# Peilun-Tommy-Li/pHNN-MPC

Measured on AMD Instinct MI355X. Metric: pHNN-MPC rollouts+grads/sec, cartpole H=50 batch=65536, higher is better.
Workload: dtype f32

## Files before the change

phnn_mpc_amd/csrc/phnn_kernels.hip.h:

```cpp
#pragma once
#include <hip/hip_runtime.h>

#include "../../include/phnn_mpc.h"

#define DEV __device__ __forceinline__
#ifdef PHNN_CACHED_TAPE
#define PHNN_NT_STORE(v, p) (*(p) = (v))
#define PHNN_NT_LOAD(p) (*(p))
#else
#define PHNN_NT_STORE(v, p) __builtin_nontemporal_store((v), (p))
#define PHNN_NT_LOAD(p) __builtin_nontemporal_load((p))
#endif

using f32x4 = __attribute__((ext_vector_type(4))) float;
using f32x2 = __attribute__((ext_vector_type(2))) float;

constexpr int kTileB = 16;
#ifndef PHNN_KMAXWAVES
#define PHNN_KMAXWAVES 8
#endif
constexpr int kMaxWaves = PHNN_KMAXWAVES;
constexpr int kScrFloats = 16 * 20;

struct Lane {
// ... 366 lines not shown
  f16x8 h[T / 2], l[T / 2];
};

template <int T>
DEV void split_act_h(const Act<T>& a, Split2<T>& o) {
#pragma unroll
  for (int s = 0; s < T / 2; ++s) {
    u32x4 H, Lo;
#pragma unroll
    for (int p = 0; p < 4; ++p) {
      f32x2 x = {a.v[2 * s + (p >> 1)][2 * (p & 1)], a.v[2 * s + (p >> 1)][2 * (p & 1) + 1]};
      f16x2 hb = __builtin_convertvector(x, f16x2);
      f32x2 r = residual_h(hb, x);
      H[p] = __builtin_bit_cast(unsigned, hb);
      Lo[p] = __builtin_bit_cast(unsigned, __builtin_convertvector(r, f16x2));
    }
    o.h[s] = __builtin_bit_cast(f16x8, H);
    o.l[s] = __builtin_bit_cast(f16x8, Lo);
  }
}

template <int HID>
struct HfImg {
  static constexpr int RS = HID + 16;
  static constexpr int PART = HID * RS * 2;
  static constexpr int FLOATS = 2 * PART / 4;
};

DEV f16x8 in_frag_h(f32x4 x) {
  f32x2 v01 = {x[0], x[1]}, v23 = {x[2], x[3]};
  f16x2 h01 = __builtin_convertvector(v01, f16x2), h23 = __builtin_convertvector(v23, f16x2);
  f32x2 r01 = residual_h(h01, v01), r23 = residual_h(h23, v23);
  u32x4 B = {__builtin_bit_cast(unsigned, h01), __builtin_bit_cast(unsigned, h23),
             __builtin_bit_cast(unsigned, __builtin_convertvector(r01, f16x2)),
             __builtin_bit_cast(unsigned, __builtin_convertvector(r23, f16x2))};
  return __builtin_bit_cast(f16x8, B);
}
constexpr int kInFragH(int T) { return T * 64 * 4; }
template <int T>
DEV void in_layer_h(Act<T>& o, const float* Wh, Lane ln, f16x8 xf) {
  keep_lds_reads_local();
#pragma unroll
  for (int nt = 0; nt < T; ++nt) o.v[nt] = mfma_h(*reinterpret_cast<const f16x8*>(Wh + (nt * 64 + ln.lane) * 4), xf, o.v[nt]);
}
constexpr int kInHFwd = 1, kInHRecomp = 2, kInHHvp = 4, kInHNet1 = 8, kInHNet1Adj = 16;
#ifndef PHNN_INH_MASK
#define PHNN_INH_MASK (kInHFwd | kInHRecomp | kInHHvp | kInHNet1 | kInHNet1Adj)
#endif
template <int T, int MM, int SITE>
DEV void in_layer_mm(Act<T>& o, const float* Lnet, int oF, int oFh, Lane ln, f32x4 x, int tile0 = 0) {
  if constexpr (MM == MM_F16X2 && (PHNN_INH_MASK & SITE) != 0) in_layer_h<T>(o, Lnet + oFh + tile0 * 256, ln, in_frag_h(x));
  else in_layer<T>(o, Lnet + oF + tile0 * 64, ln, sel4(x, ln.q));
}

DEV void mfma3x2(f32x4& o0, f32x4& o1, const f16x8 (&a)[2][2], f16x8 xh, f16x8 xl) {
  o0 = mfma_h(a[0][1], xh, o0);
  o1 = mfma_h(a[1][1], xh, o1);
  o0 = mfma_h(a[0][0], xl, o0);
  o1 = mfma_h(a[1][0], xl, o1);
  o0 = mfma_h(a[0][0], xh, o0);
  o1 = mfma_h(a[1][0], xh, o1);
}

template <int T>
DEV void sq_fwd_h(Act<T>& o, const float* Wimg, Lane ln, const Split2<T>& in) {
  using I = HfImg<16 * T>;
  keep_lds_reads_local();
  matrix_phase_begin();
  const char* base = reinterpret_cast<const char*>(Wimg) + ln.i * (I::RS * 2) + ln.q * 16;
#ifndef PHNN_NO_PREFETCH_FRAGS
  {
    constexpr int PD = 1, NB = PD + 1;
    f16x8 a[NB][2][2];
    auto loadg = [&](int g, f16x8 (&dst)[2][2]) {
      const int n0 = 2 * (g / (T / 2)), s = g % (T / 2);
#pragma unroll
      for (int gg = 0; gg < 2; ++gg)
#pragma unroll
        for (int p = 0; p < 2; ++p)
          dst[gg][p] = *reinterpret_cast<const f16x8*>(base + p * I::PART + (n0 + gg) * 16 * (I::RS * 2) + s * 64);
    };
    constexpr int NG = (T / 2) * (T / 2);
#pragma unroll
    for (int g = 0; g < PD && g < NG; ++g) loadg(g, a[g % NB]);
#pragma unroll
    for (int g = 0; g < NG; ++g) {
      if (g + PD < NG) loadg(g + PD, a[(g + PD) % NB]);
      __builtin_amdgcn_sched_barrier(0);
      const int n0 = 2 * (g / (T / 2)), s = g % (T / 2);
      mfma3x2(o.v[n0], o.v[n0 + 1], a[g % NB], in.h[s], in.l[s]);
      __builtin_amdgcn_sched_barrier(0);
    }
    matrix_phase_end();
    return;
  }
#endif
#pragma unroll
  for (int n0 = 0; n0 < T; n0 += 2) {
#pragma unroll
    for (int s = 0; s < T / 2; ++s) {
      f16x8 a[2][2];
#pragma unroll
      for (int g = 0; g < 2; ++g)
#pragma unroll
        for (int p = 0; p < 2; ++p)
          a[g][p] = *reinterpret_cast<const f16x8*>(base + p * I::PART + (n0 + g) * 16 * (I::RS * 2) + s * 64);
      mfma3x2(o.v[n0], o.v[n0 + 1], a, in.h[s], in.l[s]);
    }
  }
  matrix_phase_end();
}

template <int T>
DEV void sq_bwd_h(Act<T>& o, const float* Wimg, Lane ln, const Split2<T>& in) {
  using I = HfImg<16 * T>;
  keep_lds_reads_local();
  matrix_phase_begin();
  typedef fp16x4_t __attribute__((address_space(3))) * lds_h4;
  typedef char __attribute__((address_space(3))) * lds_cp;
  const int a4 = (ln.lane & 15) >> 2, pp = ln.lane & 3;
  lds_cp base = (lds_cp) const_cast<char*>(reinterpret_cast<const char*>(Wimg)) + (4 * ln.q + a4) * (I::RS * 2) + 16 * pp;
#ifndef PHNN_NO_PREFETCH_FRAGS
  {
    f16x8 a[2][2][2];
    auto loadg = [&](int g, f16x8 (&dst)[2][2]) {
      const int n0 = 2 * (g / (T / 2)), s = g % (T / 2);
#pragma unroll
      for (int gg = 0; gg < 2; ++gg) {
        const int nt = n0 + gg;
#pragma unroll
        for (int p = 0; p < 2; ++p) {
          lds_cp off = base + p * I::PART + 32 * s * (I::RS * 2) + (64 * (nt >> 1) + 8 * (nt & 1));
          f16x4 lo = __builtin_bit_cast(f16x4, __builtin_amdgcn_ds_read_tr16_b64_v4f16((lds_h4)off));
          f16x4 hi = __builtin_bit_cast(f16x4, __builtin_amdgcn_ds_read_tr16_b64_v4f16((lds_h4)(off + 16 * (I::RS * 2))));
          dst[gg][p] = __builtin_shufflevector(lo, hi, 0, 1, 2, 3, 4, 5, 6, 7);
        }
      }
    };
    constexpr int NG = (T / 2) * (T / 2);
    constexpr int PD = 1, NB = PD + 1;
#pragma unroll
    for (int g = 0; g < PD && g < NG; ++g) loadg(g, a[g % NB]);
#pragma unroll
    for (int g = 0; g < NG; ++g) {
      if (g + PD < NG) loadg(g + PD, a[(g + PD) % NB]);
      __builtin_amdgcn_sched_barrier(0);
      const int n0 = 2 * (g / (T / 2)), s = g % (T / 2);
      mfma3x2(o.v[n0], o.v[n0 + 1], a[g % NB], in.h[s], in.l[s]);
      __builtin_amdgcn_sched_barrier(0);
    }
    matrix_phase_end();
    return;
  }
#endif
#pragma unroll
  for (int n0 = 0; n0 < T; n0 += 2) {
#pragma unroll
    for (int s = 0; s < T / 2; ++s) {
      f16x8 a[2][2];
#pragma unroll
      for (int g = 0; g < 2; ++g) {
        const int nt = n0 + g;
#pragma unroll
        for (int p = 0; p < 2; ++p) {
          lds_cp off = base + p * I::PART + 32 * s * (I::RS * 2) + (64 * (nt >> 1) + 8 * (nt & 1));
          f16x4 lo = __builtin_bit_cast(f16x4, __builtin_amdgcn_ds_read_tr16_b64_v4f16((lds_h4)off));
          f16x4 hi = __builtin_bit_cast(f16x4, __builtin_amdgcn_ds_read_tr16_b64_v4f16((lds_h4)(off + 16 * (I::RS * 2))));
          a[g][p] = __builtin_shufflevector(lo, hi, 0, 1, 2, 3, 4, 5, 6, 7);
        }
      }
      mfma3x2(o.v[n0], o.v[n0 + 1], a, in.h[s], in.l[s]);
    }
  }
  matrix_phase_end();
}

template <int TG>
DEV f32x4 to4_group(const float* Wt_group, Lane ln, const f32x4* in_tiles) {
  const float* base = Wt_group + 4 * ln.q;
  f32x4 o0 = splat4(0.f), o1 = splat4(0.f);
#pragma unroll
  for (int t = 0; t < TG; ++t) {
    f32x4 a = *reinterpret_cast<const f32x4*>(base + 16 * t);
#pragma unroll
    for (int r = 0; r < 4; ++r) {
      if ((r & 1) == 0) o0 = __builtin_amdgcn_mfma_f32_4x4x1f32(a[r], in_tiles[t][r], o0, 0, 0, 0);
      else o1 = __builtin_amdgcn_mfma_f32_4x4x1f32(a[r], in_tiles[t][r], o1, 0, 0, 0);
    }
  }
  return o0 + o1;
}

DEV f32x4 to4_kslots(f32x4 o) {
#ifdef PHNN_BPERMUTE_REDUCE
#pragma unroll
  for (int c = 0; c < 4; ++c) {
    float v = o[c];
    v += __shfl_xor(v, 16);
    v += __shfl_xor(v, 32);
    o[c] = v;
  }
  return o;
#else
  f32x4 b;
  asm volatile("v_mov_b32 %4, %0\n\tv_mov_b32 %5, %1\n\tv_mov_b32 %6, %2\n\tv_mov_b32 %7, %3\n\t"
               "v_permlane16_swap_b32 %0, %4\n\tv_permlane16_swap_b32 %1, %5\n\t"
               "v_permlane16_swap_b32 %2, %6\n\tv_permlane16_swap_b32 %3, %7\n\ts_nop 0"
               : "+v"(o[0]), "+v"(o[1]), "+v"(o[2]), "+v"(o[3]), "=&v"(b[0]), "=&v"(b[1]), "=&v"(b[2]), "=&v"(b[3]));
  o = o + b;
  asm volatile("v_mov_b32 %4, %0\n\tv_mov_b32 %5, %1\n\tv_mov_b32 %6, %2\n\tv_mov_b32 %7, %3\n\t"
               "v_permlane32_swap_b32 %0, %4\n\tv_permlane32_swap_b32 %1, %5\n\t"
               "v_permlane32_swap_b32 %2, %6\n\tv_permlane32_swap_b32 %3, %7\n\ts_nop 0"
               : "+v"(o[0]), "+v"(o[1]), "+v"(o[2]), "+v"(o[3]), "=&v"(b[0]), "=&v"(b[1]), "=&v"(b[2]), "=&v"(b[3]));
  return o + b;
#endif
}

template <int TI>
DEV f32x4 to4_rep(const float* Wt, Lane ln, const Act<TI>& in) {
  constexpr int LR = 16 * TI + 8;
  keep_lds_reads_local();
  const float* row = Wt + (ln.i & 3) * LR;
  constexpr int TG = TI >= 2 ? 2 : 1, NG = TI / TG;
  f32x4 tot = to4_group<TG>(row, ln, &in.v[0]);
#pragma unroll
  for (int g = 1; g < NG; ++g) tot = tot + to4_group<TG>(row + 16 * TG * g, ln, &in.v[TG * g]);
  return to4_kslots(tot);
}

template <int T>
DEV void store_act(float* dst, Lane ln, const Act<T>& a) {
#pragma unroll
  for (int t = 0; t < T; ++t) PHNN_NT_STORE(a.v[t], reinterpret_cast<f32x4*>(dst) + t * 64 + ln.lane);
}
template <int T>
DEV void load_act(const float* src, Lane ln, Act<T>& a) {
#pragma unroll
  for (int t = 0; t < T; ++t) {
#ifdef PHNN_PLAIN_STASH_LOADS
    a.v[t] = reinterpret_cast<const f32x4*>(src)[t * 64 + ln.lane];
#else
    a.v[t] = PHNN_NT_LOAD(reinterpret_cast<const f32x4*>(src) + t * 64 + ln.lane);
#endif
  }
}

constexpr float kFix24 = 8388607.0f;
typedef unsigned u32x3 __attribute__((ext_vector_type(3), aligned(4)));
template <int T>
DEV void store_act24(float* dst, Lane ln, const Act<T>& a) {
#pragma unroll
  for (int t = 0; t < T; ++t) {
    unsigned q[4];
#pragma unroll
    for (int r = 0; r < 4; ++r) q[r] = (unsigned)(int)__builtin_rintf(a.v[t][r] * kFix24);
    u32x3 d = {__builtin_amdgcn_perm(q[1], q[0], 0x04020100u),
               __builtin_amdgcn_perm(q[2], q[1], 0x05040201u),
               __builtin_amdgcn_perm(q[3], q[2], 0x06050402u)};
    PHNN_NT_STORE(d, reinterpret_cast<u32x3*>(reinterpret_cast<char*>(dst) + (t * 64 + ln.lane) * 12));
  }
}
template <int T>
DEV void load_act24(const float* src, Lane ln, Act<T>& a) {
#pragma unroll
  for (int t = 0; t < T; ++t) {
    const u32x3 d = PHNN_NT_LOAD(reinterpret_cast<const u32x3*>(reinterpret_cast<const char*>(src) + (t * 64 + ln.lane) * 12));
    const int q0 = (int)(d[0] << 8) >> 8;
    const int q1 = (int)(__builtin_amdgcn_alignbit(d[1], d[0], 24) << 8) >> 8;
    const int q2 = (int)(__builtin_amdgcn_alignbit(d[2], d[1], 16) << 8) >> 8;
    const int q3 = (int)d[2] >> 8;
    a.v[t] = f32x4{(float)q0, (float)q1, (float)q2, (float)q3} * (1.0f / kFix24);
  }
}

DEV void gather16(float* scr, Lane ln, f32x4 mine, float (&out)[16]) {
  float* row = scr + ln.i * 20;
  *reinterpret_cast<f32x4*>(row + 4 * ln.q) = mine;
  __builtin_amdgcn_wave_barrier();
#pragma unroll
  for (int k = 0; k < 4; ++k) {
    f32x4 v = *reinterpret_cast<const f32x4*>(row + 4 * k);
    out[4 * k + 0] = v[0];
    out[4 * k + 1] = v[1];
    out[4 * k + 2] = v[2];
    out[4 * k + 3] = v[3];
  }
  __builtin_amdgcn_wave_barrier();
}

DEV float reduce_q(float v) {
#ifdef PHNN_BPERMUTE_REDUCE
  v += __shfl_xor(v, 16);
  v += __shfl_xor(v, 32);
  return v;
#else
  float b;
  asm volatile("v_mov_b32 %1, %0\n\ts_nop 1\n\tv_permlane16_swap_b32 %0, %1\n\ts_nop 0" : "+v"(v), "=&v"(b));
  v += b;
  asm volatile("v_mov_b32 %1, %0\n\ts_nop 1\n\tv_permlane32_swap_b32 %0, %1\n\ts_nop 0" : "+v"(v), "=&v"(b));
  return v + b;
#endif
}


template <int HID, int MM = MM_F32>
struct LayH2 {
  static constexpr int T = HID / 16, LD = HID + 4, LR = HID + 8;
  static constexpr int oW2 = 0;
  static constexpr int W2F = MM == MM_F32 ? HID * LD : (MM == MM_BF16X3 ? BfImg<HID>::FLOATS : HfImg<HID>::FLOATS);
  static constexpr int oW1h = oW2 + W2F;
  static constexpr int oW1f = oW1h + (MM == MM_F16X2 ? T * 64 * 4 : 0);
  static constexpr int oB1 = oW1f + T * 64;
  static constexpr int oB2 = oB1 + HID;
  static constexpr int oW3 = oB2 + HID;
  static constexpr int oW3B = oW3 + HID;
  static constexpr int oW3S = oW3B + HID;
  static constexpr int oW1T = oW3S + HID;
  static constexpr int oB3 = oW1T + 4 * LR;
  static constexpr int SIZE = oB3 + 4;
};

template <int HID, int MM = MM_F32>
struct LayH1 {
  static constexpr int T = HID / 16, LD = HID + 4, LR = HID + 8;
  static constexpr bool HF = MM == MM_F16X2;
  static constexpr int RS = HID + 16;
  static constexpr int FPART = 16 * RS * 2;
  static constexpr int BPART = HID * 16 * 2;
  static constexpr int oV2 = 0;
  static constexpr int oV2T = oV2 + 2 * FPART / 4;
  static constexpr int V2F = HF ? (2 * FPART + 2 * BPART) / 4 : 16 * LD;
  static constexpr int oV1h = oV2 + V2F;
  static constexpr int oV1f = oV1h + (HF ? T * 64 * 4 : 0);
  static constexpr int oC1 = oV1f + T * 64;
  static constexpr int oC2 = oC1 + HID;
  static constexpr int oSc = oC2 + 16;
  static constexpr int oV1T = oSc + 4;
  static constexpr int SIZE = oV1T + 4 * LR;
};

constexpr int kRecSmall = 40;
template <int T, int NBIG>
struct WRec {
  static constexpr int VEC = T * 256;
  static constexpr int oSmall = NBIG * VEC;
  static constexpr int SIZE = oSmall + 16 * kRecSmall;
};

#ifdef PHNN_CACHED_RECORDS
#define PHNN_REC_STORE(v, p) (*(p) = (v))
#define PHNN_REC_LOAD(p) (*(p))
#else
#define PHNN_REC_STORE(v, p) __builtin_nontemporal_store((v), (p))
#define PHNN_REC_LOAD(p) __builtin_nontemporal_load((p))
#endif
template <int T>
DEV void store_rec(float* dst, Lane ln, const Act<T>& a) {
#pragma unroll
  for (int t = 0; t < T; ++t) PHNN_REC_STORE(a.v[t], reinterpret_cast<f32x4*>(dst) + t * 64 + ln.lane);
}
template <int T>
DEV void store_rec_scaled(float* dst, Lane ln, const Act<T>& a, float s) {
#pragma unroll
  for (int t = 0; t < T; ++t) PHNN_REC_STORE(a.v[t] * s, reinterpret_cast<f32x4*>(dst) + t * 64 + ln.lane);
}

constexpr int ACT_TANH = 0, ACT_SILU = 2, ACT_RELU = 3, ACT_ELU = 4, ACT_GELU = 5;

DEV float gelu_pdf(float z) { return 0.3989422804014327f * __builtin_amdgcn_exp2f(z * z * -0.7213475204444817f); }
DEV float gelu_cdf(float z) { return __builtin_fmaf(0.5f, erff(z * 0.7071067811865476f), 0.5f); }

template <int ACT>
DEV void act_eval(float z, float& a, float& d1) {
  if (ACT == ACT_RELU) {
    a = fmaxf(z, 0.f);
    d1 = z > 0.f ? 1.0f : 0.0f;
  } else if (ACT == ACT_ELU) {
    a = z > 0.f ? z : expm1f(z);
    d1 = z > 0.f ? 1.0f : __builtin_amdgcn_exp2f(z * 1.4426950408889634f);
  } else if (ACT == ACT_GELU) {
    const float c = gelu_cdf(z);
    a = z * c;
    d1 = __builtin_fmaf(z, gelu_pdf(z), c);
  } else {
    const float s = __builtin_amdgcn_rcpf(1.0f + __builtin_amdgcn_exp2f(z * -1.4426950408889634f));
    a = z * s;
    d1 = __builtin_fmaf(a, 1.0f - s, s);
  }
}
template <int ACT>
DEV float act_d2(float z) {
  if (ACT == ACT_RELU) return 0.0f;
  if (ACT == ACT_ELU) return z > 0.f ? 0.0f : __builtin_amdgcn_exp2f(z * 1.4426950408889634f);
  if (ACT == ACT_GELU) return gelu_pdf(z) * __builtin_fmaf(-z, z, 2.0f);
  const float s = __builtin_amdgcn_rcpf(1.0f + __builtin_amdgcn_exp2f(z * -1.4426950408889634f));
  return s * (1.0f - s) * __builtin_fmaf(z, 1.0f - 2.0f * s, 2.0f);
}
template <int ACT, int T>
DEV void act_of(const Act<T>& z, Act<T>& a) {
#pragma unroll
  for (int t = 0; t < T; ++t)
#pragma unroll
    for (int r = 0; r < 4; ++r) {
      float av, d;
      act_eval<ACT>(z.v[t][r], av, d);
      a.v[t][r] = av;
    }
}
template <int ACT, int T>
DEV void mul_d1(Act<T>& g, const Act<T>& z) {
#pragma unroll
  for (int t = 0; t < T; ++t)
#pragma unroll
    for (int r = 0; r < 4; ++r) {
      float a, d;
      act_eval<ACT>(z.v[t][r], a, d);
      g.v[t][r] *= d;
    }
}

template <int HID>
struct HTape {
  Act<HID / 16> a1, a2, q1;
};

template <int HID, bool WANT_H, int ACT>
DEV f32x4 hnet_grad_g(const float* L, Lane ln, f32x4 x, HTape<HID>& tp, float& Hval) {
  using Y = LayH2<HID, MM_F32>;
  constexpr int T = Y::T;
  load_vec<T>(tp.a1, L + Y::oB1, ln);
  in_layer<T>(tp.a1, L + Y::oW1f, ln, sel4(x, ln.q));
  {
    Act<T> a;
    act_of<ACT, T>(tp.a1, a);
    load_vec<T>(tp.a2, L + Y::oB2, ln);
    sq_fwd<T, T>(tp.a2, L + Y::oW2, ln, a);
  }
  Act<T> g;
  float s = 0.f;
  keep_lds_reads_local();
#pragma unroll
  for (int t = 0; t < T; ++t) {
    f32x4 w3 = *reinterpret_cast<const f32x4*>(L + Y::oW3 + 16 * t + 4 * ln.q);
#pragma unroll
    for (int r = 0; r < 4; ++r) {
      float a, d;
      act_eval<ACT>(tp.a2.v[t][r], a, d);
      if (WANT_H) s = __builtin_fmaf(w3[r], a, s);
      g.v[t][r] = w3[r] * d;
    }
  }
  if (WANT_H) Hval = reduce_q(s) + L[Y::oB3];
  zero_act<T>(tp.q1);
  sq_bwd<T, T>(tp.q1, L + Y::oW2, ln, g);
#pragma unroll
  for (int t = 0; t < T; ++t) g.v[t] = tp.q1.v[t];
  mul_d1<ACT, T>(g, tp.a1);
  return to4_rep<T>(L + Y::oW1T, ln, g);
}
template <int HID, int ACT>
DEV void hnet_layer1_g(const float* L, Lane ln, f32x4 x, Act<HID / 16>& z1) {
  using Y = LayH2<HID, MM_F32>;
  load_vec<Y::T>(z1, L + Y::oB1, ln);
  in_layer<Y::T>(z1, L + Y::oW1f, ln, sel4(x, ln.q));
}
template <int HID, int ACT>
DEV f32x4 hnet_hvp_g(const float* L, Lane ln, HTape<HID>& tp, f32x4 v) {
  using Y = LayH2<HID, MM_F32>;
  constexpr int T = Y::T;
  Act<T> ad1, w;
  zero_act<T>(ad1);
  in_layer<T>(ad1, L + Y::oW1f, ln, sel4(v, ln.q));
#pragma unroll
  for (int t = 0; t < T; ++t)
#pragma unroll
    for (int r = 0; r < 4; ++r) {
      const float z = tp.a1.v[t][r], zd = ad1.v[t][r];
      float a, d;
      act_eval<ACT>(z, a, d);
      tp.q1.v[t][r] = tp.q1.v[t][r] * (act_d2<ACT>(z) * zd);
      ad1.v[t][r] = d * zd;
    }
  zero_act<T>(w);
  sq_fwd<T, T>(w, L + Y::oW2, ln, ad1);
  keep_lds_reads_local();
#pragma unroll
  for (int t = 0; t < T; ++t) {
    f32x4 w3 = *reinterpret_cast<const f32x4*>(L + Y::oW3 + 16 * t + 4 * ln.q);
#pragma unroll
    for (int r = 0; r < 4; ++r) w.v[t][r] = w3[r] * (act_d2<ACT>(tp.a2.v[t][r]) * w.v[t][r]);
  }
  Act<T> qd;
  zero_act<T>(qd);
  sq_bwd<T, T>(qd, L + Y::oW2, ln, w);
  mul_d1<ACT, T>(qd, tp.a1);
#pragma unroll
  for (int t = 0; t < T; ++t) qd.v[t] = qd.v[t] + tp.q1.v[t];
  return to4_rep<T>(L + Y::oW1T, ln, qd);
}

template <int HID, bool WANT_H, int MM = MM_F32, int SITE = kInHFwd, int ACT = ACT_TANH>
DEV f32x4 hnet_grad(const float* L, Lane ln, f32x4 z, HTape<HID>& tp, float& Hval) {
  if constexpr (ACT != ACT_TANH) {
    static_assert(MM == MM_F32, "SiLU / ReLU run on the all-f32 kernels");
    return hnet_grad_g<HID, WANT_H, ACT>(L, ln, z, tp, Hval);
  }
  using Y = LayH2<HID, MM>;
  constexpr int T = Y::T;
  load_vec<T>(tp.a1, L + Y::oB1, ln);
  in_layer_mm<T, MM, SITE>(tp.a1, L, Y::oW1f, Y::oW1h, ln, z);
  tanh_act_pre<T>(tp.a1);
  load_vec<T>(tp.a2, L + Y::oB2, ln);
  if (MM == MM_BF16X3) {
    Split3<T> sp;
    split_act<T>(tp.a1, sp);
    sq_fwd_bf<T>(tp.a2, L + Y::oW2, ln, sp);
  } else if (MM == MM_F16X2) {
    Split2<T> sp;
    split_act_h<T>(tp.a1, sp);
    sq_fwd_h<T>(tp.a2, L + Y::oW2, ln, sp);
  } else {
    sq_fwd<T, T>(tp.a2, L + Y::oW2, ln, tp.a1);
  }
  if (MM == MM_F16X2 || kPreScaled<T>) {
    const float c = L[Y::oB3 + 1];
    if (kPreScaled<T> && c == 1.0f) {
      tanh_act_pre<T>(tp.a2);
    } else {
#pragma unroll
      for (int t = 0; t < T; ++t)
#pragma unroll
        for (int r = 0; r < 4; ++r) tp.a2.v[t][r] = tanh_scaled(tp.a2.v[t][r], c);
    }
  } else {
    tanh_act<T>(tp.a2);
  }
  Act<T> g;
  float s = 0.f;
  keep_lds_reads_local();
#pragma unroll
  for (int t = 0; t < T; ++t) {
    if (WANT_H) {
      f32x4 w3 = *reinterpret_cast<const f32x4*>(L + Y::oW3 + 16 * t + 4 * ln.q);
#pragma unroll
      for (int r = 0; r < 4; ++r) s = __builtin_fmaf(w3[r], tp.a2.v[t][r], s);
    }
    f32x4 w3b = *reinterpret_cast<const f32x4*>(L + Y::oW3B + 16 * t + 4 * ln.q);
    g.v[t] = w3b * dtanh(tp.a2.v[t]);
  }
  if (WANT_H) Hval = reduce_q(s) + L[Y::oB3];
  zero_act<T>(tp.q1);
  if (MM == MM_BF16X3) {
    Split3<T> sp;
    split_act<T>(g, sp);
    sq_bwd_bf<T>(tp.q1, L + Y::oW2, ln, sp);
  } else if (MM == MM_F16X2) {
    Split2<T> sp;
    split_act_h<T>(g, sp);
    sq_bwd_h<T>(tp.q1, L + Y::oW2, ln, sp);
  } else {
    sq_bwd<T, T>(tp.q1, L + Y::oW2, ln, g);
  }
#pragma unroll
  for (int t = 0; t < T; ++t) g.v[t] = tp.q1.v[t] * dtanh(tp.a1.v[t]);
  return to4_rep<T>(L + Y::oW1T, ln, g);
}

template <int HID, int MM, int ACT = ACT_TANH>
DEV void hnet_layer1(const float* L, Lane ln, f32x4 z, Act<HID / 16>& a1) {
  if constexpr (ACT != ACT_TANH) return hnet_layer1_g<HID, ACT>(L, ln, z, a1);
  using Y = LayH2<HID, MM>;
  load_vec<Y::T>(a1, L + Y::oB1, ln);
  in_layer_mm<Y::T, MM, kInHRecomp>(a1, L, Y::oW1f, Y::oW1h, ln, z);
  tanh_act_pre<Y::T>(a1);
}

template <int HID, int MM = MM_F32, bool WG = false, int ACT = ACT_TANH>
DEV f32x4 hnet_hvp(const float* L, Lane ln, HTape<HID>& tp, f32x4 v, float* rec = nullptr) {
  if constexpr (ACT != ACT_TANH) {
    static_assert(!WG, "weight-gradient kernels exist for Tanh models only");
    return hnet_hvp_g<HID, ACT>(L, ln, tp, v);
  }
  using Y = LayH2<HID, MM>;
  constexpr int T = Y::T;
  float unscale = 1.0f;
  if (MM == MM_F16X2) {
    float mx = fmaxf(fmaxf(__builtin_fabsf(v[0]), __builtin_fabsf(v[1])), fmaxf(__builtin_fabsf(v[2]), __builtin_fabsf(v[3])));
    int e = 0;
    (void)__builtin_frexpf(mx, &e);
    e = (mx > 0.f && mx < 3.0e38f) ? e : 0;
    v = v * __builtin_ldexpf(1.0f, -e);
    unscale = __builtin_ldexpf(1.0f, e);
  }
  Act<T> ad1, w;
  zero_act<T>(ad1);
  in_layer_mm<T, MM, kInHHvp>(ad1, L, Y::oW1f, Y::oW1h, ln, v);
#pragma unroll
  for (int t = 0; t < T; ++t) ad1.v[t] = dtanh(tp.a1.v[t]) * ad1.v[t];
#pragma unroll
  for (int t = 0; t < T; ++t) tp.q1.v[t] = tp.q1.v[t] * (tp.a1.v[t] * ad1.v[t]);
  zero_act<T>(w);
  if (MM == MM_BF16X3) {
    Split3<T> sp;
    split_act<T>(ad1, sp);
    sq_fwd_bf<T>(w, L + Y::oW2, ln, sp);
  } else if (MM == MM_F16X2) {
    Split2<T> sp;
    split_act_h<T>(ad1, sp);
    sq_fwd_h<T>(w, L + Y::oW2, ln, sp);
  } else {
    sq_fwd<T, T>(w, L + Y::oW2, ln, ad1);
  }
  keep_lds_reads_local();
#pragma unroll
  for (int t = 0; t < T; ++t) {
    f32x4 w3 = *reinterpret_cast<const f32x4*>(L + Y::oW3S + 16 * t + 4 * ln.q);
    f32x4 a2 = tp.a2.v[t];
    f32x4 ad2 = dtanh(a2) * w.v[t];
    if (WG) PHNN_REC_STORE(ad2 * unscale, reinterpret_cast<f32x4*>(rec + 2 * T * 256) + t * 64 + ln.lane);
    w.v[t] = w3 * (a2 * ad2);
  }
  Act<T> qd;
  zero_act<T>(qd);
  if (MM == MM_BF16X3) {
    Split3<T> sp;
    split_act<T>(w, sp);
    sq_bwd_bf<T>(qd, L + Y::oW2, ln, sp);
  } else if (MM == MM_F16X2) {
    Split2<T> sp;
    split_act_h<T>(w, sp);
    sq_bwd_h<T>(qd, L + Y::oW2, ln, sp);
  } else {
    sq_bwd<T, T>(qd, L + Y::oW2, ln, w);
  }
  if (WG) store_rec_scaled<T>(rec + 3 * T * 256, ln, qd, unscale);
#pragma unroll
  for (int t = 0; t < T; ++t) {
    qd.v[t] = __builtin_elementwise_fma(qd.v[t], dtanh(tp.a1.v[t]), tp.q1.v[t]);
  }
  f32x4 Hv = to4_rep<T>(L + Y::oW1T, ln, qd);
  return Hv * (-2.0f * unscale * L[Y::oB3 + 2]);
}

template <int HID, int MM>
DEV f32x4 h1_out_hf(const float* L, Lane ln, const Split2<HID / 16>& sp) {
  using Y = LayH1<HID, MM>;
  constexpr int T = Y::T;
  keep_lds_reads_local();
  const char* base = reinterpret_cast<const char*>(L + Y::oV2) + ln.i * (Y::RS * 2) + ln.q * 16;
  f32x4 o0 = splat4(0.f), o1 = splat4(0.f), o2 = splat4(0.f);
#pragma unroll
  for (int s = 0; s < T / 2; ++s) {
    f16x8 ah = *reinterpret_cast<const f16x8*>(base + s * 64);
    f16x8 al = *reinterpret_cast<const f16x8*>(base + Y::FPART + s * 64);
    o0 = mfma_h(al, sp.h[s], o0);
    o1 = mfma_h(ah, sp.l[s], o1);
    o2 = mfma_h(ah, sp.h[s], o2);
  }
  const float inv = L[Y::oSc];
  f32x4 c2 = *reinterpret_cast<const f32x4*>(L + Y::oC2 + 4 * ln.q);
  return ((o0 + o1) + o2) * inv + c2;
}

template <int HID, int MM>
DEV void h1_bwd_operands(const float* L, Lane ln, const float (&obar)[16], f16x8& b1, f16x8& b2, float& unscale) {
  using Y = LayH1<HID, MM>;
  float mx = 0.f;
#pragma unroll
  for (int k = 0; k < 16; ++k) mx = fmaxf(mx, __builtin_fabsf(obar[k]));
  int e = 0;
  (void)__builtin_frexpf(mx, &e);
  e = (mx > 0.f && mx < 3.0e38f) ? e : 0;
  const float sc = __builtin_ldexpf(1.0f, -e);
  unscale = __builtin_ldexpf(1.0f, e) * L[Y::oSc];
  const bool second = (ln.q & 1) != 0, lo_half = ln.q >= 2;
  u32x4 B1, B2;
#pragma unroll
  for (int p = 0; p < 4; ++p) {
    f32x2 v = {(second ? obar[8 + 2 * p] : obar[2 * p]) * sc, (second ? obar[9 + 2 * p] : obar[2 * p + 1]) * sc};
    f16x2 hb2 = __builtin_convertvector(v, f16x2);
    f32x2 r = residual_h(hb2, v);
    unsigned hbits = __builtin_bit_cast(unsigned, hb2), lbits = __builtin_bit_cast(unsigned, __builtin_convertvector(r, f16x2));
    B1[p] = lo_half ? lbits : hbits;
    B2[p] = lo_half ? 0u : hbits;
  }
  b1 = __builtin_bit_cast(f16x8, B1);
  b2 = __builtin_bit_cast(f16x8, B2);
}

DEV void store_rf(float* dst, Lane ln, f32x4 o) {
  if (ln.w == 0) PHNN_NT_STORE(o, reinterpret_cast<f32x4*>(dst) + ln.i * 4 + ln.q);
}
DEV void load_rf(const float* src, Lane ln, float (&rf)[16]) {
  const f32x4* p = reinterpret_cast<const f32x4*>(src) + ln.i * 4;
#pragma unroll
  for (int k = 0; k < 4; ++k) {
    f32x4 v = PHNN_NT_LOAD(p + k);
#pragma unroll
    for (int e = 0; e < 4; ++e) rf[4 * k + e] = v[e];
  }
}
template <int HID, int MM = MM_F32, int SITE = kInHNet1, int ACT = ACT_TANH>
DEV void h1_hidden(const float* L, Lane ln, f32x4 x, Act<HID / 16>& h) {
  using Y = LayH1<HID, MM>;
  constexpr int T = Y::T;
  load_vec<T>(h, L + Y::oC1, ln);
  in_layer_mm<T, MM, SITE>(h, L, Y::oV1f, Y::oV1h, ln, x);
  if constexpr (ACT == ACT_TANH) tanh_act_pre<T>(h);
}

template <int HID, int MM = MM_F32, int SITE = kInHNet1, int ACT = ACT_TANH>
DEV void h1_fwd(const float* L, float* scr, Lane ln, f32x4 x, Act<HID / 16>& h, float (&out)[16], float* rf_stash = nullptr) {
  using Y = LayH1<HID, MM>;
  constexpr int T = Y::T;
  load_vec<T>(h, L + Y::oC1, ln);
  in_layer_mm<T, MM, SITE>(h, L, Y::oV1f, Y::oV1h, ln, x);
  if constexpr (ACT != ACT_TANH) {
    static_assert(MM == MM_F32, "SiLU / ReLU run on the all-f32 kernels");
    Act<T> a;
    act_of<ACT, T>(h, a);
    Act<1> og;
    og.v[0] = *reinterpret_cast<const f32x4*>(L + Y::oC2 + 4 * ln.q);
    sq_fwd<1, T>(og, L + Y::oV2, ln, a);
    if (rf_stash) store_rf(rf_stash, ln, og.v[0]);
    gather16(scr, ln, og.v[0], out);
    return;
  }
  tanh_act_pre<T>(h);
  Act<1> o;
  if (Y::HF) {
    Split2<T> sp;
    split_act_h<T>(h, sp);
    o.v[0] = h1_out_hf<HID, MM>(L, ln, sp);
  } else {
    o.v[0] = *reinterpret_cast<const f32x4*>(L + Y::oC2 + 4 * ln.q);
    sq_fwd<1, T>(o, L + Y::oV2, ln, h);
  }
  if (rf_stash) store_rf(rf_stash, ln, o.v[0]);
  gather16(scr, ln, o.v[0], out);
}

template <int HID, int MM = MM_F32, bool WG = false, int ACT = ACT_TANH>
DEV f32x4 h1_bwd(const float* L, Lane ln, const Act<HID / 16>& h, const float (&obar)[16], float* rec = nullptr) {
  using Y = LayH1<HID, MM>;
  constexpr int T = Y::T;
  Act<T> hb;
  if constexpr (ACT != ACT_TANH) {
    static_assert(MM == MM_F32 && !WG, "SiLU / ReLU: all-f32 kernels, no weight-gradient records");
    Act<1> ob;
#pragma unroll
    for (int r = 0; r < 4; ++r)
      ob.v[0][r] = ln.q == 0 ? obar[r] : (ln.q == 1 ? obar[4 + r] : (ln.q == 2 ? obar[8 + r] : obar[12 + r]));
    zero_act<T>(hb);
    sq_bwd<T, 1>(hb, L + Y::oV2, ln, ob);
    mul_d1<ACT, T>(hb, h);
    return to4_rep<T>(L + Y::oV1T, ln, hb);
  }
  float unscale = 1.0f;
  if (Y::HF) {
    f16x8 b1, b2;
    h1_bwd_operands<HID, MM>(L, ln, obar, b1, b2, unscale);
    keep_lds_reads_local();
    const char* base = reinterpret_cast<const char*>(L + Y::oV2T) + ln.i * 32 + (ln.q & 1) * 16;
#pragma unroll
    for (int nt = 0; nt < T; ++nt) {
      f16x8 ah = *reinterpret_cast<const f16x8*>(base + nt * 512);
      f16x8 al = *reinterpret_cast<const f16x8*>(base + Y::BPART + nt * 512);
      hb.v[nt] = mfma_h(ah, b1, mfma_h(al, b2, splat4(0.f)));
    }
  } else {
    Act<1> ob;
#pragma unroll
    for (int r = 0; r < 4; ++r)
      ob.v[0][r] = ln.q == 0 ? obar[r] : (ln.q == 1 ? obar[4 + r] : (ln.q == 2 ? obar[8 + r] : obar[12 + r]));
    zero_act<T>(hb);
    sq_bwd<T, 1>(hb, L + Y::oV2, ln, ob);
  }
#pragma unroll
  for (int t = 0; t < T; ++t) hb.v[t] = hb.v[t] * dtanh(h.v[t]);
  if (WG) store_rec_scaled<T>(rec, ln, hb, Y::HF ? unscale : 1.0f);
  f32x4 xb = to4_rep<T>(L + Y::oV1T, ln, hb);
  return Y::HF ? xb * unscale : xb;
}

template <int N>
DEV void sym_from_rf(const float (&rf)[16], float (&S)[N][N]) {
#pragma unroll
  for (int i = 0; i < N; ++i) {
    S[i][i] = rf[i * N + i];
#pragma unroll
    for (int j = i + 1; j < N; ++j) S[i][j] = S[j][i] = (rf[i * N + j] + rf[j * N + i]) * 0.5f;
  }
}
template <int N>
DEV void rbar_from(f32x4 lam, f32x4 dH, const float (&Stl)[N], const float (&StdH)[N], float (&rbar)[16]) {
  float m[N][N];
#pragma unroll
  for (int k = 0; k < 16; ++k) rbar[k] = 0.f;
#pragma unroll
  for (int i = 0; i < N; ++i)
#pragma unroll
    for (int j = 0; j < N; ++j) m[i][j] = __builtin_fmaf(lam[i], StdH[j], dH[i] * Stl[j]);
#pragma unroll
  for (int i = 0; i < N; ++i) {
    rbar[i * N + i] = -m[i][i];
#pragma unroll
    for (int j = i + 1; j < N; ++j) rbar[i * N + j] = rbar[j * N + i] = (m[i][j] + m[j][i]) * -0.5f;
  }
}

template <int N_, int HID_, bool FIXG_, int MM_ = MM_F32, int MI_ = 1, int ACT_ = ACT_TANH>
struct PhnnModel {
  static constexpr int N = N_, HID = HID_, T = HID / 16, MM = MM_, MI = MI_, ACT = ACT_;
  static constexpr bool FIXG = FIXG_, SPLIT = false;
  static_assert(N_ * MI_ <= 16 && MI_ <= 4, "G_net output n*m <= 16, m <= 4");
  static constexpr int SCR = kScrFloats;
  static constexpr int oH = 0;
  static constexpr int oR = oH + LayH2<HID, MM>::SIZE;
  static constexpr int oGn = oR + LayH1<HID, MM>::SIZE;
  static constexpr int oJ = oGn + (FIXG ? 0 : LayH1<HID, MM>::SIZE);
  static constexpr int oG = oJ + 16;
  static constexpr int IMG = oG + 16;

  static constexpr int oStashRf = 2 * T * 256 + 64;
  static constexpr int STASH = oStashRf + 256;

  template <bool WANT_H, bool ST = false>
  DEV static f32x4 f(const float* L, float* scr, Lane ln, f32x4 x, f32x4 u, float& Hval, float* stash = nullptr) {
    keep_lds_reads_local();
    HTape<HID> tp;
    f32x4 dH = hnet_grad<HID, WANT_H, MM, kInHFwd, ACT>(L + oH, ln, x, tp, Hval);
    if (ST) {
      store_act<T>(stash, ln, tp.a2);
      store_act<T>(stash + T * 256, ln, tp.q1);
      if (ln.q == 0) PHNN_NT_STORE(dH, reinterpret_cast<f32x4*>(stash + 2 * T * 256) + ln.i);
    }
    Act<T> hR;
    float rf[16];
    h1_fwd<HID, MM, kInHNet1, ACT>(L + oR, scr, ln, x, hR, rf, ST ? stash + oStashRf : nullptr);
    float G[N * MI];
    if (FIXG) {
#pragma unroll
      for (int i = 0; i < N * MI; ++i) G[i] = L[oG + i];
    } else {
      Act<T> hG;
      float gf[16];
      h1_fwd<HID, MM, kInHNet1, ACT>(L + oGn, scr, ln, x, hG, gf);
#pragma unroll
      for (int i = 0; i < N * MI; ++i) G[i] = gf[i];
    }
    return combine(L, rf, dH, G, u);
  }

  DEV static f32x4 combine(const float* L, const float (&rf)[16], f32x4 dH, const float (&G)[N * MI], f32x4 u) {
    float S[N][N], StdH[N];
    sym_from_rf<N>(rf, S);
#pragma unroll
    for (int k = 0; k < N; ++k) {
      float a = 0.f;
#pragma unroll
      for (int i = 0; i < N; ++i) a = __builtin_fmaf(S[i][k], dH[i], a);
      StdH[k] = a;
    }
    f32x4 dx = splat4(0.f);
#pragma unroll
    for (int i = 0; i < N; ++i) {
      float acc = 0.f;
#pragma unroll
      for (int j = 0; j < N; ++j) acc = __builtin_fmaf(L[oJ + i * N + j], dH[j], acc);
#pragma unroll
      for (int k = 0; k < N; ++k) acc = __builtin_fmaf(-S[i][k], StdH[k], acc);
      if (MI == 1) {
        dx[i] = __builtin_fmaf(G[i], u[0], acc);
      } else {
        float gu = 0.f;
#pragma unroll
        for (int k = 0; k < MI; ++k) gu = __builtin_fmaf(G[i * MI + k], u[k], gu);
        dx[i] = acc + gu;
      }
    }
    return dx;
  }

  static constexpr bool RECHB = !LayH1<HID, MM>::HF;
  static constexpr int NBIG = 4 + (RECHB ? (FIXG ? 1 : 2) : 0);
  using Rec = WRec<T, NBIG>;

  template <bool ST = false, bool WG = false>
  DEV static void vjp(const float* L, float* scr, Lane ln, f32x4 x, f32x4 u, f32x4 lam, f32x4& xbar, f32x4& ubar,
                      const float* stash = nullptr, float* rec = nullptr, float Hbar = 0.f) {
    keep_lds_reads_local();
    HTape<HID> tp;
    float Hdummy;
    f32x4 dH;
    float rf[16];
    if (ST) {
      dH = PHNN_NT_LOAD(reinterpret_cast<const f32x4*>(stash + 2 * T * 256) + ln.i);
      load_rf(stash + oStashRf, ln, rf);
      load_act<T>(stash, ln, tp.a2);
      load_act<T>(stash + T * 256, ln, tp.q1);
    } else {
      dH = hnet_grad<HID, false, MM, kInHRecomp, ACT>(L + oH, ln, x, tp, Hdummy);
    }
    if (WG && !ST) {
      store_rec<T>(rec, ln, tp.a2);
      store_rec<T>(rec + Rec::VEC, ln, tp.q1);
    }
    f32x4 xb = splat4(0.f);
    float S[N][N], Stl[N], StdH[N];
    {
      Act<T> hR;
      if (ST) {
        h1_hidden<HID, MM, kInHNet1Adj, ACT>(L + oR, ln, x, hR);
      } else {
        h1_fwd<HID, MM, kInHNet1Adj, ACT>(L + oR, scr, ln, x, hR, rf);
      }
      sym_from_rf<N>(rf, S);
#pragma unroll
      for (int k = 0; k < N; ++k) {
        float a = 0.f, c = 0.f;
#pragma unroll
        for (int i = 0; i < N; ++i) {
          a = __builtin_fmaf(S[i][k], lam[i], a);
          c = __builtin_fmaf(S[i][k], dH[i], c);
        }
        Stl[k] = a;
        StdH[k] = c;
      }
      float rbar[16];
      rbar_from<N>(lam, dH, Stl, StdH, rbar);
      xb += h1_bwd<HID, MM, WG && RECHB, ACT>(L + oR, ln, hR, rbar, WG && RECHB ? rec + 4 * Rec::VEC : nullptr);
      if (WG && ln.q == 0) {
        f32x4* sm = reinterpret_cast<f32x4*>(rec + Rec::oSmall + ln.i * kRecSmall);
#pragma unroll
        for (int k = 0; k < 4; ++k) sm[4 + k] = f32x4{rbar[4 * k], rbar[4 * k + 1], rbar[4 * k + 2], rbar[4 * k + 3]};
      }
    }
    ubar = splat4(0.f);
    if (FIXG) {
#pragma unroll
      for (int k = 0; k < MI; ++k)
#pragma unroll
        for (int i = 0; i < N; ++i) ubar[k] = __builtin_fmaf(L[oG + i * MI + k], lam[i], ubar[k]);
    } else {
      Act<T> hG;
      float gf[16], gbar[16];
      h1_fwd<HID, MM, kInHNet1Adj, ACT>(L + oGn, scr, ln, x, hG, gf);
#pragma unroll
      for (int k = 0; k < 16; ++k) gbar[k] = 0.f;
#pragma unroll
      for (int i = 0; i < N; ++i)
#pragma unroll
        for (int k = 0; k < MI; ++k) {
          ubar[k] = __builtin_fmaf(gf[i * MI + k], lam[i], ubar[k]);
          gbar[i * MI + k] = lam[i] * u[k];
        }
      xb += h1_bwd<HID, MM, WG && RECHB, ACT>(L + oGn, ln, hG, gbar, WG && RECHB ? rec + 5 * Rec::VEC : nullptr);
    }
    f32x4 v = splat4(0.f);
#pragma unroll
    for (int j = 0; j < N; ++j) {
      float acc = 0.f;
#pragma unroll
      for (int i = 0; i < N; ++i) acc = __builtin_fmaf(L[oJ + i * N + j], lam[i], acc);
#pragma unroll
      for (int k = 0; k < N; ++k) acc = __builtin_fmaf(-S[j][k], Stl[k], acc);
      v[j] = acc;
    }
    if (WG && ln.q == 0) {
      f32x4* sm = reinterpret_cast<f32x4*>(rec + Rec::oSmall + ln.i * kRecSmall);
      sm[0] = x;
      sm[1] = v;
      sm[2] = lam;
      sm[3] = dH;
      sm[8] = u;
      sm[9] = f32x4{Hbar, 0.f, 0.f, 0.f};
    }
    if (ST) hnet_layer1<HID, MM, ACT>(L + oH, ln, x, tp.a1);
    xbar = xb + hnet_hvp<HID, MM, WG, ACT>(L + oH, ln, tp, v, rec);
    if (WG) xbar = xbar + Hbar * dH;
  }
};

struct LayM {
  static constexpr int HID = 64, T = 4, LD = HID + 4, LR = HID + 8;
  static constexpr int oW1f = 0;
  static constexpr int oB1 = oW1f + T * 64;
  static constexpr int oW2 = oB1 + HID;
  static constexpr int oB2 = oW2 + HID * LD;
  static constexpr int oWo = oB2 + HID;
  static constexpr int oBo = oWo + 4 * LR;
  static constexpr int oWoTf = oBo + 4;
  static constexpr int oW1T = oWoTf + T * 64;
  static constexpr int SIZE = oW1T + 4 * LR;
};

struct MTape {
  Act<4> a1, a2;
  f32x4 o;
};

DEV void mnet_fwd(const float* L, Lane ln, f32x4 q, MTape& tp) {
  using Y = LayM;
  keep_lds_reads_local();
  load_vec<4>(tp.a1, L + Y::oB1, ln);
  in_layer<4>(tp.a1, L + Y::oW1f, ln, sel4(q, ln.q));
  tanh_act<4>(tp.a1);
  load_vec<4>(tp.a2, L + Y::oB2, ln);
  sq_fwd<4, 4>(tp.a2, L + Y::oW2, ln, tp.a1);
  tanh_act<4>(tp.a2);
  tp.o = to4_rep<4>(L + Y::oWo, ln, tp.a2) + *reinterpret_cast<const f32x4*>(L + Y::oBo);
}

DEV f32x4 mnet_bwd(const float* L, Lane ln, const MTape& tp, f32x4 ob) {
  using Y = LayM;
  keep_lds_reads_local();
  Act<4> d, e;
  zero_act<4>(d);
  in_layer<4>(d, L + Y::oWoTf, ln, sel4(ob, ln.q));
#pragma unroll
  for (int t = 0; t < 4; ++t) d.v[t] = d.v[t] * dtanh(tp.a2.v[t]);
  zero_act<4>(e);
  sq_bwd<4, 4>(e, L + Y::oW2, ln, d);
#pragma unroll
  for (int t = 0; t < 4; ++t) e.v[t] = e.v[t] * dtanh(tp.a1.v[t]);
  return to4_rep<4>(L + Y::oW1T, ln, e);
}

DEV float softplus_dev(float x) { return x > 20.f ? x : log1pf(expf(x)); }
DEV float sigmoid_sp_dev(float x) { return x > 20.f ? 1.0f : 1.0f / (1.0f + expf(-x)); }

constexpr int MASS_CARTPOLE = 0, MASS_CONSTANT = 1, MASS_DIAGONAL = 2, MASS_FULL = 3;

template <int MT>
DEV void mass_from_outputs(f32x4 o, float (&m)[3], float (&w)[3]) {
  if (MT == MASS_DIAGONAL) {
    m[0] = expf(o[0]) + 1e-3f;
    m[2] = expf(o[1]) + 1e-3f;
    m[1] = 0.f;
    w[0] = 1.0f / m[0];
    w[2] = 1.0f / m[2];
    w[1] = 0.f;
  } else {
    const float l00 = softplus_dev(o[0]) + 1e-3f, l10 = o[1], l11 = softplus_dev(o[2]) + 1e-3f;
    m[0] = l00 * l00;
    m[1] = l00 * l10;
    m[2] = l10 * l10 + l11 * l11;
    const float det = m[0] * m[2] - m[1] * m[1];
    w[0] = m[2] / det;
    w[1] = -m[1] / det;
    w[2] = m[0] / det;
  }
}

template <int MT>
DEV f32x4 mass_outputs_bar(f32x4 o, const float (&Mb)[4]) {
  if (MT == MASS_DIAGONAL) return f32x4{Mb[0] * expf(o[0]), Mb[3] * expf(o[1]), 0.f, 0.f};
  const float l00 = softplus_dev(o[0]) + 1e-3f, l10 = o[1], l11 = softplus_dev(o[2]) + 1e-3f;
  const float s00 = 2.0f * Mb[0], s01 = Mb[1] + Mb[2], s11 = 2.0f * Mb[3];
  return f32x4{(s00 * l00 + s01 * l10) * sigmoid_sp_dev(o[0]), s01 * l00 + s11 * l10, (s11 * l11) * sigmoid_sp_dev(o[2]), 0.f};
}

template <int HID_, int MM_ = MM_F32, int MI_ = 1, int MT_ = MASS_CARTPOLE, int ACT_ = ACT_TANH>
struct CanonModel {
  static constexpr int N = 4, HID = HID_, T = HID / 16, MM = MM_, MI = MI_, MT = MT_, ACT = ACT_;
  static constexpr bool SPLIT = false;
  static constexpr int SCR = 0;
  static constexpr int oH = 0;
  static constexpr int oC = oH + LayH2<HID, MM>::SIZE;
  static constexpr int oCG = oC + 12;
  static constexpr int oCW = oC + 28;
  static constexpr int oMn = oC + 32;
  static constexpr int IMG = oMn + (MT_ >= MASS_DIAGONAL ? LayM::SIZE : 0);

  DEV static void mass_eval(const float* L, Lane ln, f32x4 y, float (&m)[3], float (&w)[3], MTape& mt) {
    if (MT == MASS_CONSTANT) {
      m[0] = L[oC + 0]; m[1] = L[oC + 1]; m[2] = L[oC + 2];
      w[0] = L[oCW + 0]; w[1] = L[oCW + 1]; w[2] = L[oCW + 2];
    } else {
      mnet_fwd(L + oMn, ln, f32x4{y[0], y[1], 0.f, 0.f}, mt);
      mass_from_outputs<MT>(mt.o, m, w);
    }
  }

  DEV static float Base_Gu(const float* L, int row, f32x4 u) {
    float s = 0.f;
#pragma unroll
    for (int k = 0; k < MI; ++k) s = __builtin_fmaf(L[oCG + row * MI + k], u[k], s);
    return s;
  }
  DEV static f32x4 Base_Gt(const float* L, float dpb0, float dpb1) {
    f32x4 ub = splat4(0.f);
#pragma unroll
    for (int k = 0; k < MI; ++k) ub[k] = L[oCG + 2 * MI + k] * dpb0 + L[oCG + 3 * MI + k] * dpb1;
    return ub;
  }

  static constexpr int STASH = 2 * T * 256 + 64;

  template <bool WANT_H, bool ST = false>
  DEV static f32x4 f(const float* L, float* scr, Lane ln, f32x4 y, f32x4 u, float& Hval, float* stash = nullptr) {
    keep_lds_reads_local();
    if constexpr (MT != MASS_CARTPOLE) {
      float m[3], w[3];
      MTape mt;
      mass_eval(L, ln, y, m, w, mt);
      f32x4 z = {y[0], y[1], m[0] * y[2] + m[1] * y[3], m[1] * y[2] + m[2] * y[3]};
      HTape<HID> tp;
      f32x4 dH = hnet_grad<HID, WANT_H, MM, kInHFwd, ACT>(L + oH, ln, z, tp, Hval);
      if (ST) {
        store_act<T>(stash, ln, tp.a2);
        store_act<T>(stash + T * 256, ln, tp.q1);
        if (ln.q == 0) PHNN_NT_STORE(dH, reinterpret_cast<f32x4*>(stash + 2 * T * 256) + ln.i);
      }
      float dp0 = (-dH[0] - L[oC + 6] * dH[2]) + Base_Gu(L, 2, u);
      float dp1 = (-dH[1] - L[oC + 7] * dH[3]) + Base_Gu(L, 3, u);
      return f32x4{w[0] * z[2] + w[1] * z[3], w[1] * z[2] + w[2] * z[3], w[0] * dp0 + w[1] * dp1, w[1] * dp0 + w[2] * dp1};
    }
    float a = L[oC + 0], b = L[oC + 1], c = L[oC + 2];
    float sn, cs;
    sincos_dev(y[1], sn, cs);
    float bc = b * cs;
    f32x4 z = {y[0], y[1], a * y[2] + bc * y[3], bc * y[2] + c * y[3]};
    HTape<HID> tp;
    f32x4 dH = hnet_grad<HID, WANT_H, MM, kInHFwd, ACT>(L + oH, ln, z, tp, Hval);
    if (ST) {
      store_act<T>(stash, ln, tp.a2);
      store_act<T>(stash + T * 256, ln, tp.q1);
      if (ln.q == 0) PHNN_NT_STORE(dH, reinterpret_cast<f32x4*>(stash + 2 * T * 256) + ln.i);
    }
    float dp0 = (-dH[0] - L[oC + 6] * dH[2]) + Base_Gu(L, 2, u);
    float dp1 = (-dH[1] - L[oC + 7] * dH[3]) + Base_Gu(L, 3, u);
    float det = (a * c - bc * bc) + 1e-6f;
    float mi00 = c / det, mi01 = -bc / det, mi11 = a / det;
    return f32x4{mi00 * z[2] + mi01 * z[3], mi01 * z[2] + mi11 * z[3], mi00 * dp0 + mi01 * dp1,
                 mi01 * dp0 + mi11 * dp1};
  }

  static constexpr int NBIG = 4;
  using Rec = WRec<T, NBIG>;

  template <bool ST = false, bool WG = false>
  DEV static void vjp(const float* L, float* scr, Lane ln, f32x4 y, f32x4 u, f32x4 lam, f32x4& ybar, f32x4& ubar,
                      const float* stash = nullptr, float* rec = nullptr, float Hbar = 0.f) {
    keep_lds_reads_local();
    if constexpr (MT != MASS_CARTPOLE) {
      float m[3], w[3];
      MTape mt;
      mass_eval(L, ln, y, m, w, mt);
      f32x4 z = {y[0], y[1], m[0] * y[2] + m[1] * y[3], m[1] * y[2] + m[2] * y[3]};
      HTape<HID> tp;
      float Hdummy;
      f32x4 dH;
      if (ST) {
        dH = PHNN_NT_LOAD(reinterpret_cast<const f32x4*>(stash + 2 * T * 256) + ln.i);
        load_act<T>(stash, ln, tp.a2);
        load_act<T>(stash + T * 256, ln, tp.q1);
        hnet_layer1<HID, MM, ACT>(L + oH, ln, z, tp.a1);
      } else {
        dH = hnet_grad<HID, false, MM, kInHRecomp, ACT>(L + oH, ln, z, tp, Hdummy);
      }
      const float Rd2 = L[oC + 6], Rd3 = L[oC + 7];
      const float dp0 = (-dH[0] - Rd2 * dH[2]) + Base_Gu(L, 2, u);
      const float dp1 = (-dH[1] - Rd3 * dH[3]) + Base_Gu(L, 3, u);
      const float pb0 = lam[0] * w[0] + lam[1] * w[1], pb1 = lam[0] * w[1] + lam[1] * w[2];
      const float dpb0 = lam[2] * w[0] + lam[3] * w[1], dpb1 = lam[2] * w[1] + lam[3] * w[2];
      f32x4 v = {-dpb0, -dpb1, -Rd2 * dpb0, -Rd3 * dpb1};
      ubar = Base_Gt(L, dpb0, dpb1);
      if (WG) {
        if (!ST) {
          store_rec<T>(rec, ln, tp.a2);
          store_rec<T>(rec + Rec::VEC, ln, tp.q1);
        }
        if (ln.q == 0) {
          f32x4* sm = reinterpret_cast<f32x4*>(rec + Rec::oSmall + ln.i * kRecSmall);
          sm[0] = z;
          sm[1] = v;
          sm[2] = lam;
          sm[3] = dH;
          sm[4] = f32x4{0.f, 0.f, -dpb0 * dH[2], -dpb1 * dH[3]};
          sm[8] = u;
          sm[9] = f32x4{Hbar, 0.f, 0.f, 0.f};
        }
// ... 1679 lines not shown
```

Baseline: 31.20 million.

## Distribute small S/G algebra across quarter-waves instead of replicating per lane

```diff
diff --git a/phnn_mpc_amd/csrc/phnn_kernels.hip.h b/phnn_mpc_amd/csrc/phnn_kernels.hip.h
--- a/phnn_mpc_amd/csrc/phnn_kernels.hip.h
+++ b/phnn_mpc_amd/csrc/phnn_kernels.hip.h
@@ -692,6 +692,39 @@
 #endif
 }
 
+#ifdef PHNN_REPLICATED_SMALLALG
+constexpr bool kOwnedSmallAlg = false;
+#else
+constexpr bool kOwnedSmallAlg = true;
+#endif
+DEV f32x4 allgather_q(Lane ln, float a) {
+#ifdef PHNN_BPERMUTE_REDUCE
+  return f32x4{__shfl(a, ln.i), __shfl(a, 16 + ln.i), __shfl(a, 32 + ln.i), __shfl(a, 48 + ln.i)};
+#else
+  float b, c, d;
+  asm("v_mov_b32 %1, %0\n\ts_nop 1\n\tv_permlane16_swap_b32 %0, %1\n\ts_nop 0" : "+v"(a), "=&v"(b));
+  asm("v_mov_b32 %2, %0\n\tv_mov_b32 %3, %1\n\ts_nop 1\n\t"
+               "v_permlane32_swap_b32 %0, %2\n\tv_permlane32_swap_b32 %1, %3\n\ts_nop 0"
+               : "+v"(a), "+v"(b), "=&v"(c), "=&v"(d));
+  return f32x4{a, b, c, d};
+#endif
+}
+DEV void publish16(float* scr, Lane ln, f32x4 mine) {
+  *reinterpret_cast<f32x4*>(scr + ln.i * 20 + 4 * ln.q) = mine;
+  __builtin_amdgcn_wave_barrier();
+}
+template <int CNT>
+DEV void read16(const float* scr, Lane ln, int first, int stride, float (&out)[CNT]) {
+  const float* row = scr + ln.i * 20 + first;
+#pragma unroll
+  for (int k = 0; k < CNT; ++k) out[k] = row[k * stride];
+}
+template <int N>
+DEV void sym_row(const float (&row)[N], const float (&col)[N], float (&Sq)[N]) {
+#pragma unroll
+  for (int j = 0; j < N; ++j) Sq[j] = (row[j] + col[j]) * 0.5f;
+}
+
 
 template <int HID, int MM = MM_F32>
 struct LayH2 {
@@ -1100,7 +1133,7 @@
 }
 
 template <int HID, int MM = MM_F32, int SITE = kInHNet1, int ACT = ACT_TANH>
-DEV void h1_fwd(const float* L, float* scr, Lane ln, f32x4 x, Act<HID / 16>& h, float (&out)[16], float* rf_stash = nullptr) {
+DEV f32x4 h1_fwd_mine(const float* L, Lane ln, f32x4 x, Act<HID / 16>& h, float* rf_stash = nullptr) {
   using Y = LayH1<HID, MM>;
   constexpr int T = Y::T;
   load_vec<T>(h, L + Y::oC1, ln);
@@ -1113,8 +1146,7 @@
     og.v[0] = *reinterpret_cast<const f32x4*>(L + Y::oC2 + 4 * ln.q);
     sq_fwd<1, T>(og, L + Y::oV2, ln, a);
     if (rf_stash) store_rf(rf_stash, ln, og.v[0]);
-    gather16(scr, ln, og.v[0], out);
-    return;
+    return og.v[0];
   }
   tanh_act_pre<T>(h);
   Act<1> o;
@@ -1127,7 +1159,11 @@
     sq_fwd<1, T>(o, L + Y::oV2, ln, h);
   }
   if (rf_stash) store_rf(rf_stash, ln, o.v[0]);
-  gather16(scr, ln, o.v[0], out);
+  return o.v[0];
+}
+template <int HID, int MM = MM_F32, int SITE = kInHNet1, int ACT = ACT_TANH>
+DEV void h1_fwd(const float* L, float* scr, Lane ln, f32x4 x, Act<HID / 16>& h, float (&out)[16], float* rf_stash = nullptr) {
+  gather16(scr, ln, h1_fwd_mine<HID, MM, SITE, ACT>(L, ln, x, h, rf_stash), out);
 }
 
 template <int HID, int MM = MM_F32, bool WG = false, int ACT = ACT_TANH>
@@ -1226,6 +1262,24 @@
       if (ln.q == 0) PHNN_NT_STORE(dH, reinterpret_cast<f32x4*>(stash + 2 * T * 256) + ln.i);
     }
     Act<T> hR;
+    if constexpr (kOwnedSmallAlg) {
+      float row[N], col[N], Sq[N], Gq[MI];
+      publish16(scr, ln, h1_fwd_mine<HID, MM, kInHNet1, ACT>(L + oR, ln, x, hR, ST ? stash + oStashRf : nullptr));
+      read16<N>(scr, ln, ln.q * N, 1, row);
+      read16<N>(scr, ln, ln.q, N, col);
+      __builtin_amdgcn_wave_barrier();
+      sym_row<N>(row, col, Sq);
+      if (FIXG) {
+#pragma unroll
+        for (int k = 0; k < MI; ++k) Gq[k] = L[oG + ln.q * MI + k];
+      } else {
+        Act<T> hG;
+        publish16(scr, ln, h1_fwd_mine<HID, MM, kInHNet1, ACT>(L + oGn, ln, x, hG));
+        read16<MI>(scr, ln, ln.q * MI, 1, Gq);
+        __builtin_amdgcn_wave_barrier();
+      }
+      return combine_owned(L, ln, Sq, dH, Gq, u);
+    }
     float rf[16];
     h1_fwd<HID, MM, kInHNet1, ACT>(L + oR, scr, ln, x, hR, rf, ST ? stash + oStashRf : nullptr);
     float G[N * MI];
@@ -1269,6 +1323,31 @@
         dx[i] = acc + gu;
       }
     }
+    return dx;
+  }
+
+  DEV static f32x4 combine_owned(const float* L, Lane ln, const float (&Sq)[N], f32x4 dH, const float (&Gq)[MI], f32x4 u) {
+    float a = 0.f;
+#pragma unroll
+    for (int i = 0; i < N; ++i) a = __builtin_fmaf(Sq[i], dH[i], a);
+    const f32x4 StdH = allgather_q(ln, a);
+    float acc = 0.f;
+#pragma unroll
+    for (int j = 0; j < N; ++j) acc = __builtin_fmaf(L[oJ + ln.q * N + j], dH[j], acc);
+#pragma unroll
+    for (int k = 0; k < N; ++k) acc = __builtin_fmaf(-Sq[k], StdH[k], acc);
+    float dq;
+    if (MI == 1) {
+      dq = __builtin_fmaf(Gq[0], u[0], acc);
+    } else {
+      float gu = 0.f;
+#pragma unroll
+      for (int k = 0; k < MI; ++k) gu = __builtin_fmaf(Gq[k], u[k], gu);
+      dq = acc + gu;
+    }
+    f32x4 dx = allgather_q(ln, dq);
+#pragma unroll
+    for (int i = N; i < 4; ++i) dx[i] = 0.f;
     return dx;
   }
 
```

After: 31.31 million (median of 6 runs). Within noise of the previous version (+0.4%).
